# tqch/v-diffusion-torch

Hardware: AMD Instinct MI355X
Metric: train_images_per_sec (higher is better)
Workload: dtype fp32 (bf16x3 split products in the tile-engine GEMMs)

## Files before the change

v-diffusion-torch_amd/csrc/common.h:

```cpp
#pragma once
#include <hip/hip_runtime.h>
#include <stdint.h>
#include <stdio.h>
#include "../../include/vdiff_hip.h"

typedef float f32x4 __attribute__((ext_vector_type(4)));
typedef float f32x16 __attribute__((ext_vector_type(16)));

typedef float f32x2 __attribute__((ext_vector_type(2)));

#ifdef VD_PROBES
constexpr bool VD_PROBE_BUILD = true;
#else
constexpr bool VD_PROBE_BUILD = false;
#endif

void vd_set_error(const char* fmt, ...);
int vd_cu_count(void);
int vd_persistent_cus(void);
int vd_gemm_grouped_wgrad_kblk(const float* const* A, const float* const* B, float* const* C, float* const* colsum, int32_t count, int32_t M,
                               int32_t N, int32_t K, int64_t lda, int64_t ldb, int64_t ldc, int32_t splitk, float* ws, size_t ws_bytes,
                               void* stream, int64_t a_kblk, int64_t b_kblk, int32_t slabs_only);
int vd_gemm_grouped_wgrad_used_slabs(int32_t count, int32_t M, int32_t N, int32_t K, int32_t splitk);
int vd_gemm_rowblk(const vd_gemm_desc* d, int64_t a_rblk, void* stream);
// ... 14 lines not shown
__device__ __forceinline__ float vd_sigmoid(float x) { return __builtin_amdgcn_rcpf(1.0f + __expf(-x)); }

__device__ __forceinline__ void vd_philox4(uint64_t seed, uint64_t ctr, uint32_t out[4]) {
    uint32_t k0 = (uint32_t)seed, k1 = (uint32_t)(seed >> 32);
    uint32_t c0 = (uint32_t)ctr, c1 = (uint32_t)(ctr >> 32), c2 = 0x243F6A88u, c3 = 0x85A308D3u;
#pragma unroll
    for (int r = 0; r < 10; ++r) {
        uint64_t p0 = (uint64_t)0xD2511F53u * c0, p1 = (uint64_t)0xCD9E8D57u * c2;
        uint32_t n0 = (uint32_t)(p1 >> 32) ^ c1 ^ k0, n2 = (uint32_t)(p0 >> 32) ^ c3 ^ k1;
        c1 = (uint32_t)p1; c3 = (uint32_t)p0; c0 = n0; c2 = n2;
        k0 += 0x9E3779B9u; k1 += 0xBB67AE85u;
    }
    out[0] = c0; out[1] = c1; out[2] = c2; out[3] = c3;
}
__device__ __forceinline__ f32x4 vd_dropout_scale4(uint64_t seed, uint64_t vec_index, float p) {
    uint32_t r[4];
    vd_philox4(seed, vec_index, r);
    const float inv = 1.0f / (1.0f - p);
    f32x4 m;
#pragma unroll
    for (int j = 0; j < 4; ++j) m[j] = ((r[j] >> 8) * (1.0f / 16777216.0f) >= p) ? inv : 0.0f;
    return m;
}
```

v-diffusion-torch_amd/csrc/norm.hip:

```cpp
#include "common.h"
#include <stdlib.h>

namespace {

constexpr int PPC = 128;

template <bool NT>
__device__ __forceinline__ f32x4 ld_stream(const float* p) {
    if (NT) return __builtin_nontemporal_load(reinterpret_cast<const f32x4*>(p));
    return *reinterpret_cast<const f32x4*>(p);
}
template <bool NT>
__device__ __forceinline__ void st_stream(float* p, f32x4 v) {
    if (NT) __builtin_nontemporal_store(v, reinterpret_cast<f32x4*>(p));
    else *reinterpret_cast<f32x4*>(p) = v;
}

struct ReduceArgs {
    const float* x; long long ldx;
    const float* dy; long long lddy;
    const float* coef;
    int act; float p_drop; unsigned long long seed; int resample; int has_norm;
    int H, W;
    long long HW;
// ... 176 lines not shown
    const int b = idx / C, c = idx % C, g = c / (C / G);
    const float mean = stats[2 * (b * G + g)], rstd = stats[2 * (b * G + g) + 1];
    float sc = rstd * gamma[c];
    float of = beta[c] - mean * sc;
    if (film) {
        const float shift = film[(long long)b * 2 * C + c], scale = film[(long long)b * 2 * C + C + c];
        sc *= (1.f + scale);
        of = of * (1.f + scale) + shift;
    }
    float* o = coef + (long long)b * 4 * C + c;
    o[0] = sc; o[C] = of; o[2 * C] = rstd; o[3 * C] = -mean * rstd;
}

struct ApplyArgs {
    const float* x; long long ldx; const float* coef; int has_norm; int act; float p_drop; unsigned long long seed;
    int resample; float* y; long long ldy; int nimg, H, W, C;
};
struct PartArgs {
    const float* p1; int C1, ch1; const float* p2; int C2, ch2; int G; float eps;
    const float* gamma; const float* beta; const float* film; float* coef_out;
};

__device__ __forceinline__ f32x4 fwd_val(const ApplyArgs& p, f32x4 v, int pix, int c4, f32x4 sc, f32x4 of, int b) {
    if (p.has_norm) v = v * sc + of;
    if (p.act) {
#pragma unroll
        for (int j = 0; j < 4; ++j) v[j] = v[j] * vd_sigmoid(v[j]);
    }
    if (p.p_drop > 0.f) {
        const unsigned long long vi = ((unsigned long long)b * p.H * p.W + pix) * (p.C >> 2) + (c4 >> 2);
        v *= vd_dropout_scale4(p.seed, vi, p.p_drop);
    }
    return v;
}
__device__ __forceinline__ f32x4 fwd_one(const ApplyArgs& p, const float* ximg, int pix, int c4, f32x4 sc, f32x4 of, int b) {
    return fwd_val(p, *reinterpret_cast<const f32x4*>(ximg + (long long)pix * p.ldx + c4), pix, c4, sc, of, b);
}

constexpr int APIX = 64;

template <bool FROM_PARTS>
__global__ __launch_bounds__(256) void gn_apply_kernel(const ApplyArgs p, int Cb, const PartArgs q) {
    __shared__ double ps[FROM_PARTS ? 2 : 1][FROM_PARTS ? 1024 : 1];
    __shared__ float gst[FROM_PARTS ? 2 : 1][FROM_PARTS ? 256 : 1];
    const int b = blockIdx.y, c0 = blockIdx.z * Cb;
    const int cbw = min(Cb, p.C - c0);
    const int vecs = cbw >> 2, rows = 256 / vecs;
    const int r = threadIdx.x / vecs, c4 = c0 + 4 * (threadIdx.x % vecs);
    const int Ho = p.resample == VD_RS_DOWN ? p.H >> 1 : (p.resample == VD_RS_UP ? p.H << 1 : p.H);
    const int Wo = p.resample == VD_RS_DOWN ? p.W >> 1 : (p.resample == VD_RS_UP ? p.W << 1 : p.W);
    const int p0 = blockIdx.x * APIX, np = min(APIX, Ho * Wo - p0);
    f32x4 sc = {1.f, 1.f, 1.f, 1.f}, of = {0.f, 0.f, 0.f, 0.f};
    if (FROM_PARTS) {
        const int C = p.C, cg = C / q.G;
        for (int cl = threadIdx.x; cl < cbw; cl += 256) {
            const int c = c0 + cl;
// ... 746 lines not shown
```

v-diffusion-torch_amd/csrc/wino43.hip:

```cpp
#include "common.h"
#include "../../include/vdiff_hip_dgrad_planes.h"
#include <stdlib.h>
#include <type_traits>

namespace {

typedef __attribute__((address_space(3))) void* lds_ptr_t;
constexpr unsigned OOB = 0x80000000u;
constexpr int KT = 8;
constexpr int TN = 32;
constexpr int TILES = 64;
constexpr int U_STAGE = 36 * 4 * 16 * 2 * 2;
constexpr int THREADS = 512;

struct Args43 {
    const float* x; long long ldx;
    const float* U;
    float* y; long long ldy;
    int nimg, H, W, K, N;
    int items_per_img;
    int ngrp;
    int ncb, nitems;
    const float* bias; const float* res; long long ldr;
    float* stats;
// ... 473 lines not shown
    o[3] = e2 + f2;
    o[4] = e2 - f2;
    o[5] = 1.265625f * d[1] + (d[5] - 2.8125f * d[3]);
}
__device__ __forceinline__ void a6(const f32x4 (&y)[4], f32x4 (&o)[6]) {
    const f32x4 e1 = y[0] + 0.5625f * y[2], f1 = 0.75f * y[1] + 0.421875f * y[3];
    const f32x4 e2 = y[0] + 2.25f * y[2], f2 = 1.5f * y[1] + 3.375f * y[3];
    o[0] = y[0];
    o[1] = e1 + f1;
    o[2] = e1 - f1;
    o[3] = e2 + f2;
    o[4] = e2 - f2;
    o[5] = y[3];
}

__device__ __forceinline__ void st_once(float* p, f32x4 v) { *reinterpret_cast<f32x4*>(p) = v; }
struct WgT43 {
    const float* x; long long ldx; const float* dy; long long lddy;
    float* V; float* dM;
    int nimg, H, W, Cin, Cout, TW, TPI, T;
    int z0;
};

__global__ __launch_bounds__(256) void wino43_wgrad_transform_kernel(const WgT43 p) {
    const int quad = blockIdx.y * 64 + threadIdx.x, tile = blockIdx.x * 4 + threadIdx.y;
    if (tile >= p.T) return;
    const int img = tile / p.TPI, tin = tile - img * p.TPI;
    const int ty = tin / p.TW, tx = tin - ty * p.TW;
    const int c4 = 4 * quad;
    if ((int)blockIdx.z + p.z0 == 0) {
        if (c4 >= p.Cin) return;
        f32x4 R[6][6];
#pragma unroll
        for (int pr = 0; pr < 6; ++pr) {
            const int yy = 4 * ty - 1 + pr;
            f32x4 d[6];
#pragma unroll
            for (int q = 0; q < 6; ++q) {
                const int xx = 4 * tx - 1 + q;
                d[q] = f32x4{0.f, 0.f, 0.f, 0.f};
                if ((unsigned)yy < (unsigned)p.H && (unsigned)xx < (unsigned)p.W)
                    d[q] = *reinterpret_cast<const f32x4*>(p.x + ((long long)(img * p.H + yy) * p.W + xx) * p.ldx + c4);
            }
            bt6(d, R[pr]);
        }
#pragma unroll
        for (int b = 0; b < 6; ++b) {
            f32x4 col[6], o[6];
#pragma unroll
            for (int pr = 0; pr < 6; ++pr) col[pr] = R[pr][b];
            bt6(col, o);
#pragma unroll
            for (int a = 0; a < 6; ++a)
                st_once(p.V + ((long long)((tile >> 4) * 36 + 6 * a + b) * 16 + (tile & 15)) * p.Cin + c4, o[a]);
        }
    } else {
        if (c4 >= p.Cout) return;
        f32x4 R[4][6];
#pragma unroll
        for (int u = 0; u < 4; ++u) {
            f32x4 y[4];
#pragma unroll
            for (int v = 0; v < 4; ++v)
                y[v] = *reinterpret_cast<const f32x4*>(p.dy + ((long long)(img * p.H + 4 * ty + u) * p.W + 4 * tx + v) * p.lddy + c4);
            a6(y, R[u]);
        }
#pragma unroll
        for (int b = 0; b < 6; ++b) {
            const f32x4 col[4] = {R[0][b], R[1][b], R[2][b], R[3][b]};
            f32x4 o[6];
            a6(col, o);
#pragma unroll
            for (int a = 0; a < 6; ++a)
                st_once(p.dM + ((long long)((tile >> 4) * 36 + 6 * a + b) * 16 + (tile & 15)) * p.Cout + c4, o[a]);
        }
    }
}

__global__ __launch_bounds__(256) void wino43_wgrad_finish_kernel(const float* dU, const float* cs, int Cout, int Cin, int Cout_w, int Cin_w,
                                                                  float* dw, float* dbias, int accumulate) {
    const long long idx = (long long)blockIdx.x * blockDim.x + threadIdx.x;
    if (dbias && idx < Cout_w) {
        const double pv[6] = {-1.0 / 9, 8.0 / 9, 0.0, 2.0 / 9, 0.0, -1.0 / 8};
        double c = 0.0;
#pragma unroll
        for (int a = 0; a < 6; ++a)
#pragma unroll
            for (int b = 0; b < 6; ++b)
                if (pv[a] != 0.0 && pv[b] != 0.0) c += pv[a] * pv[b] * (double)cs[(long long)(6 * a + b) * Cout + idx];
        dbias[idx] = accumulate ? dbias[idx] + (float)c : (float)c;
    }
    if (idx >= (long long)Cout * Cin) return;
    const int co = (int)(idx / Cin), ci = (int)(idx - (long long)co * Cin);
    if (co >= Cout_w || ci >= Cin_w) return;
    float u[6][6];
#pragma unroll
    for (int a = 0; a < 6; ++a)
#pragma unroll
        for (int b = 0; b < 6; ++b) u[a][b] = dU[(long long)(6 * a + b) * Cout * Cin + idx];
// ... 504 lines not shown
    if (T >= (1LL << 22) || 36LL * 16 * Cin * 16 + 16LL * Cin + 256 >= 0x70000000LL / 4) return 0;
    if (128LL * Cin + 128 >= 0x70000000LL / 4 || 128LL * Cout + 128 >= 0x70000000LL / 4) return 0;
    return 1;
}

extern "C" size_t vd_conv3x3_wino43_v_floats(int32_t nimg, int32_t H, int32_t W, int32_t Cin) {
    return (size_t)36 * ((size_t)nimg * (H / 4) * (W / 4)) * Cin;
}

extern "C" size_t vd_conv3x3_wino43_fwd_planes_ws_bytes(int32_t nimg, int32_t H, int32_t W, int32_t Cin, int32_t Cout) {
    const size_t T = (size_t)nimg * (H / 4) * (W / 4);
    return ((size_t)36 * Cout * Cin + (size_t)36 * T * Cout) * sizeof(float);
}

extern "C" int vd_conv3x3_fwd_planes_preferred(int32_t nimg, int32_t H, int32_t W, int32_t Cin, int32_t Cout, int32_t training) {
    if (!vd_conv3x3_wino43_fwd_planes_supported(nimg, H, W, Cin, Cout, Cin, Cout, Cout)) return 0;
    const long long T = (long long)nimg * (H / 4) * (W / 4);
    static const long long floor_t = getenv("VD_PLANES_MIN_TILES") ? atoll(getenv("VD_PLANES_MIN_TILES")) : VD_PLANES_MIN_TILES;
    static const int inference = getenv("VD_PLANES_INFERENCE") ? atoi(getenv("VD_PLANES_INFERENCE")) : VD_PLANES_INFERENCE;
    if (T < floor_t || Cout % 256 || Cin % 16) return 0;
    return training ? VD_PLANES_TRAINING : (inference != 0);
}

extern "C" int vd_conv3x3_wino43_fwd_planes(const float* xin, int64_t ldx, const float* w_oihw, const float* bias, const float* res,
                                            int64_t ldres, float* y, int64_t ldy, int32_t nimg, int32_t H, int32_t W, int32_t Cin,
                                            int32_t Cout, float* stats_part, float* V, float* ws, size_t ws_bytes, int32_t phase, void* stream) {
    VD_REQUIRE(xin && w_oihw && y && V && ws, "vd_conv3x3_wino43_fwd_planes: null operand");
    VD_REQUIRE(vd_conv3x3_wino43_fwd_planes_supported(nimg, H, W, Cin, Cout, ldx, ldy, res ? ldres : 0),
               "vd_conv3x3_wino43_fwd_planes: unsupported geometry nimg=%d H=%d W=%d Cin=%d Cout=%d", nimg, H, W, Cin, Cout);
    VD_REQUIRE(vd_aligned16(xin) && vd_aligned16(y) && vd_aligned16(V) && vd_aligned16(ws) && (!res || vd_aligned16(res)) &&
               (!bias || vd_aligned16(bias)), "vd_conv3x3_wino43_fwd_planes: operands must be 16-byte aligned");
    VD_REQUIRE(ws_bytes >= vd_conv3x3_wino43_fwd_planes_ws_bytes(nimg, H, W, Cin, Cout), "vd_conv3x3_wino43_fwd_planes: workspace too small");
    VD_REQUIRE(phase == 7 || phase == 1 || phase == 2 || phase == 4, "vd_conv3x3_wino43_fwd_planes: phase must be 7, 1, 2 or 4");
    const int TPI = (H / 4) * (W / 4), T = nimg * TPI;
    float* Up = ws;
    float* Mb = ws + (size_t)36 * Cout * Cin;
    hipStream_t st = (hipStream_t)stream;
    if (phase & 1) {
        const long long plane = (long long)Cout * Cin;
        hipLaunchKernelGGL(wino43_pack_planes_kernel, dim3((unsigned)((plane + 255) / 256)), dim3(256), 0, st, w_oihw, Up, Cout, Cin);
        VD_LAUNCH_CHECK("wino43_pack_planes_kernel");
        WgT43 t = {};
        t.x = xin; t.ldx = ldx; t.V = V;
        t.nimg = nimg; t.H = H; t.W = W; t.Cin = Cin; t.Cout = Cout; t.TW = W / 4; t.TPI = TPI; t.T = T;
        t.z0 = 0;
        hipLaunchKernelGGL(wino43_wgrad_transform_kernel, dim3((unsigned)(T / 4), (unsigned)((Cin + 255) / 256), 1), dim3(64, 4), 0, st, t);
        VD_LAUNCH_CHECK("wino43_wgrad_transform_kernel(V)");
    }
    if (phase & 2) {
        vd_gemm_desc d = {};
        d.A = V; d.B = Up; d.C = Mb;
        d.M = T; d.N = Cout; d.K = Cin; d.a_kind = VD_ROW; d.b_kind = VD_ROW;
        d.lda = Cin; d.ldb = Cin; d.ldc = Cout;
        d.batch = 36; d.nh = 1; d.alpha = 1.f;
        d.sAb = 16LL * Cin; d.sBb = (long long)Cout * Cin; d.sCb = (long long)T * Cout;
        const int rc = vd_gemm_rowblk(&d, 36LL * 16 * Cin, stream);
        if (rc) return rc;
    }
    if (phase & 4) {
        Out43 o = {};
        o.M = Mb; o.plane = (long long)T * Cout; o.bias = bias; o.res = res; o.ldr = ldres; o.y = y; o.ldy = ldy; o.stats = stats_part;
        o.H = H; o.W = W; o.Cout = Cout; o.TW = W / 4; o.TPI = TPI; o.T = T;
        o.CT = vd_conv3x3_wino43_fwd_chunk_rows(H, W) / 16;
        hipLaunchKernelGGL(wino43_out_transform_kernel, dim3((unsigned)(T / o.CT), (unsigned)((Cout + 63) / 64)), dim3(16, 16), 0, st, o);
        VD_LAUNCH_CHECK("wino43_out_transform_kernel");
    }
    return 0;
}

extern "C" size_t vd_conv3x3_wino43_dm_floats(int32_t nimg, int32_t H, int32_t W, int32_t Cout) {
    const size_t T = (size_t)nimg * (H / 4) * (W / 4);
    return (size_t)36 * ((T + 15) / 16 * 16) * Cout;
}

extern "C" int vd_conv3x3_wino43_dy_image(const float* dy, int64_t lddy, int32_t nimg, int32_t H, int32_t W, int32_t Cout, float* dM,
                                          void* stream) {
    VD_REQUIRE(dy && dM, "vd_conv3x3_wino43_dy_image: null operand");
    VD_REQUIRE(nimg > 0 && H >= 4 && W >= 4 && H % 4 == 0 && W % 4 == 0 && Cout > 0 && Cout % 4 == 0 && lddy % 4 == 0 && lddy >= Cout,
               "vd_conv3x3_wino43_dy_image: unsupported geometry nimg=%d H=%d W=%d Cout=%d", nimg, H, W, Cout);
    VD_REQUIRE(vd_aligned16(dy) && vd_aligned16(dM), "vd_conv3x3_wino43_dy_image: operands must be 16-byte aligned");
    const long long TPI = (long long)(H / 4) * (W / 4), T = nimg * TPI;
    VD_REQUIRE(T % 4 == 0 && T < (1LL << 31) && (long long)nimg * H * W * lddy < 0x7FFFFFF0LL / 4 && T * Cout * 4 < (1LL << 40),
               "vd_conv3x3_wino43_dy_image: tile count or tensor size out of range");
    WgT43 t = {};
    t.dy = dy; t.lddy = lddy; t.dM = dM;
    t.nimg = nimg; t.H = H; t.W = W; t.Cin = Cout; t.Cout = Cout; t.TW = W / 4; t.TPI = (int)TPI; t.T = (int)T;
    t.z0 = 1;
    hipLaunchKernelGGL(wino43_wgrad_transform_kernel, dim3((unsigned)(T / 4), (unsigned)((Cout + 255) / 256), 1), dim3(64, 4), 0,
                       (hipStream_t)stream, t);
    VD_LAUNCH_CHECK("wino43_wgrad_transform_kernel(dM)");
// ... 72 lines not shown
```

v-diffusion-torch_amd/v_diffusion/_hip.py:

```python
import ctypes as C
import os
import re

import numpy as np
import torch

_HERE = os.path.dirname(os.path.abspath(__file__))
HEADER_PATH = os.path.join(os.path.dirname(os.path.dirname(_HERE)), "include", "vdiff_hip.h")
LIB_PATH = os.environ.get("VDIFF_HIP_LIB") or os.path.join(os.path.dirname(_HERE), "lib", "libvdiff_hip.so")

ROW, COL, IM2COL = 0, 1, 2
TILE_WIDE = 128256
RS_NONE, RS_DOWN, RS_UP = 0, 1, 2
OUT_TYPES = {"v": 0, "x0": 1, "eps": 2, "both": 3}
REWEIGHTS = {"constant": 0, "snr": 1, "snr_trunc": 2, "snr_1plus": 3}

_i32, _i64, _f32, _vp = C.c_int32, C.c_int64, C.c_float, C.c_void_p


class GemmDesc(C.Structure):
    _fields_ = [("A", _vp), ("B", _vp), ("C", _vp), ("bias", _vp), ("R", _vp),
                ("M", _i32), ("N", _i32), ("K", _i32), ("a_kind", _i32), ("b_kind", _i32),
                ("lda", _i64), ("ldb", _i64), ("ldc", _i64), ("ldr", _i64),
                ("batch", _i32), ("nh", _i32),
# ... 35 lines not shown
        return _BY_VALUE[ctype]
    if ret not in _RETURNS:
        raise RuntimeError(f"{HEADER_PATH}: {name}: no ctypes type for the return type `{ret}`")
    return _RETURNS[ret], [arg(q) for q in params]


def _header_signatures(path=None):
    path = path or HEADER_PATH
    if not os.path.exists(path):
        raise RuntimeError(f"{path} not found: the ctypes binding is read from the C headers of the source tree")
    with open(path) as f:
        tables = _parse_header(f.read())
    return [{name: _ctypes_of(name, *decl) for name, decl in t.items()} for t in tables]


_SIGNATURES, PROBE_EXPORTS = _header_signatures()
EXPORTS = tuple(_SIGNATURES)
EXT_HEADER_PATHS = (os.path.join(os.path.dirname(HEADER_PATH), "vdiff_hip_dgrad_planes.h"),)
_EXT_SIGNATURES = {name: sig for path in EXT_HEADER_PATHS for name, sig in _header_signatures(path)[0].items()}
EXT_EXPORTS = tuple(_EXT_SIGNATURES)
DPS_HEADER_PATHS = (os.path.join(os.path.dirname(HEADER_PATH), "vdiff_hip_dps.h"),)
_DPS_SIGNATURES = {name: sig for path in DPS_HEADER_PATHS for name, sig in _header_signatures(path)[0].items()}
DPS_EXPORTS = tuple(_DPS_SIGNATURES)

_lib = None


def lib():
    global _lib
    if _lib is None:
        if not os.path.exists(LIB_PATH):
            raise RuntimeError(
                f"{LIB_PATH} not found: build it with `python __graft_entry__.py` (or make -C v-diffusion-torch_amd/csrc). "
                "The v_diffusion hot path has no CPU/PyTorch fallback.")
        l = C.CDLL(LIB_PATH)
        for name, (res, args) in {**_SIGNATURES, **_EXT_SIGNATURES, **_DPS_SIGNATURES}.items():
            fn = getattr(l, name)
            fn.restype, fn.argtypes = res, args
        for name, (res, args) in PROBE_EXPORTS.items():
            if hasattr(l, name):
                fn = getattr(l, name)
                fn.restype, fn.argtypes = res, args
        _lib = l
    return _lib


class HipError(RuntimeError):
    pass


_CPU_TENSOR = "v_diffusion HIP op received a CPU tensor: the hot path runs on an MI355X only (no CPU fallback)"


def _check(rc, what):
    if rc != 0:
        raise HipError(f"{what} failed (rc={rc}): {lib().vd_last_error().decode(errors='replace')}")


def ptr(t):
# ... 257 lines not shown
    with _TimedName(name, 2.0 * nimg * H * W * Cout * 9 * Cin):
        _check(lib().vd_conv3x3_wino43_fwd(ptr(x), ldx, ptr(U43f), ptr(bias), ptr(res), ldres, ptr(y), ldy, nimg, H, W, Cin, Cout,
                                           ptr(stats_part), stream()), "vd_conv3x3_wino43_fwd")
    _note_bytes(name, 4.0 * (nimg * H * W * (Cin + Cout + (Cout if res is not None else 0)) + 36 * Cout * Cin))


CONV_PLANES = os.environ.get("VD_CONV_PLANES", "1")


def conv3x3_fwd_planes_preferred(nimg, H, W, Cin, Cout, training):
    return bool(lib().vd_conv3x3_fwd_planes_preferred(nimg, H, W, Cin, Cout, int(bool(training))))


def conv_planes_supported(nimg, H, W, Cin, Cout, ldx, ldy, ldres=0, training=False):
    if CONV_PLANES == "0" or not (WINO and WINO43_FWD):
        return False
    if not lib().vd_conv3x3_wino43_fwd_planes_supported(nimg, H, W, Cin, Cout, ldx, ldy, ldres):
        return False
    if training and not wgrad43_supported(nimg, H, W, Cin, Cout, Cin, Cout):
        return False
    return CONV_PLANES == "2" or conv3x3_fwd_planes_preferred(nimg, H, W, Cin, Cout, training)


def conv3x3_wino43_fwd_planes(x, ldx, w, bias, y, ldy, nimg, H, W, Cin, Cout, res=None, ldres=0, stats_part=None, v=None):
    nv = lib().vd_conv3x3_wino43_v_floats(nimg, H, W, Cin)
    if v is None:
        v = workspace(nv * 4, x.device, "planes_v")
    assert v.numel() >= nv and w.is_contiguous() and tuple(w.shape) == (Cout, Cin, 3, 3)
    ws = workspace(lib().vd_conv3x3_wino43_fwd_planes_ws_bytes(nimg, H, W, Cin, Cout), x.device, "planes")
    args = (ptr(x), ldx, ptr(w), ptr(bias), ptr(res), ldres, ptr(y), ldy, nimg, H, W, Cin, Cout, ptr(stats_part), ptr(v), ws.data_ptr(),
            ws.numel() * 4)
    phase = lambda ph: _check(lib().vd_conv3x3_wino43_fwd_planes(*args, ph, stream()), "vd_conv3x3_wino43_fwd_planes")
    if PROFILE is None:
        phase(7)
        return
    T = nimg * (H // 4) * (W // 4)
    with _TimedBytes("wino43_wgrad_transform_kernel", 4.0 * nimg * H * W * Cin * (1 + 2.25)):
        phase(1)
    with _TimedTile("gemm_dma_kernel<{tile}, 0, 0, false, {kt}>", 2.0 * 36 * T * Cout * Cin):
        phase(2)
    _note_bytes(PROFILE[-1][0], 4.0 * 36.0 * (T * (Cin + Cout) + Cout * Cin))
    with _TimedBytes("wino43_out_transform_kernel", 4.0 * (36.0 * T * Cout + nimg * H * W * Cout * (2 if res is not None else 1))):
        phase(4)


DGRAD_PLANES = os.environ.get("VD_DGRAD_PLANES", "1")


def dgrad_planes_supported(nimg, H, W, Cin, Cout, lddy, lddx):
    if DGRAD_PLANES == "0" or not (WINO and WINO43):
        return False
    if lddy % 4 or not lib().vd_conv3x3_wino43_dgrad_planes_supported(nimg, H, W, Cin, Cout, lddx):
        return False
    if not wgrad43_supported(nimg, H, W, Cin, Cout, Cin, lddy):
        return False
# ... 633 lines not shown
```

v-diffusion-torch_amd/v_diffusion/engine.py:

```python
import collections
import contextlib
import math

import torch

from . import _hip as H

GROUPS = 32
EPS = 1e-6
THIN = 8


def _ld(t):
    return t.stride(2)


def _chk(t):
    B, Hh, Ww, C = t.shape
    ld = t.stride(2)
    assert t.stride(3) == 1 and t.stride(1) == Ww * ld and t.stride(0) == Hh * Ww * ld, "not an NHWC view"
    return B, Hh, Ww, C, ld


def _splitk(M, N, K, n=1):
# ... 203 lines not shown
        return torch.empty(H.stats_part_numel(nimg, HW, C), dtype=torch.float32, device=ref.device)

    @staticmethod
    def _parts(part, C, HW, rows=None):
        if part is None:
            return None
        return [(part, C, HW // (rows or (H.last_row_tile() // 2)))]

    def _norm(self, x, x_parts, gn, film, act, p_drop, seed, rs, y, B, Hh, Ww, C):
        coef = self._new(x, B, 4, C)
        stats = None
        if x_parts is not None and H.GN_FOLD and max(k for _, _, k in x_parts) <= H.GN_FOLD_MAX_CHUNKS:
            H.gn_apply_from_partials(x, _ld(x), x_parts, gn.weight, gn.bias, film, act, p_drop, seed, rs, y, _ld(y), B, Hh, Ww, C, coef,
                                     GROUPS, EPS)
            return coef
        if x_parts is not None:
            H.gn_coef_from_partials(x_parts, B, Hh * Ww, gn.weight, gn.bias, film, coef, GROUPS, EPS)
        else:
            stats = self._new(x, B, GROUPS, 2)
            H.gn_stats(x, _ld(x), B, Hh * Ww, C, stats, GROUPS, EPS)
        H.gn_apply(x, _ld(x), stats, gn.weight, gn.bias, film, act, p_drop, seed, rs, y, _ld(y), B, Hh, Ww, C, coef, GROUPS)
        return coef

    def _wgrad(self, dy, x, dw, db, M, N, K, lda, ldb, ldc):
        if self._wq is None or not H.GROUPED_WGRAD:
            H.gemm(dy, x, dw, M, N, K, a_kind=H.COL, b_kind=H.COL, lda=lda, ldb=ldb, ldc=ldc, splitk=_splitk(M, N, K), colsum=db)
            return
        key = (M, N, K, lda, ldb, ldc, db is not None)
        q = self._wq.setdefault(key, [])
        q.append((dy, x, dw, db))
        if len(q) == H.GROUP_MAX:
            self._wgrad_flush_key(key)

    def _cwgrad(self, x, ldx, dy, lddy, *args, v=None, **kw):
        if v is not None:
            kw["v"] = v
        side = self._side
        if side is None:
            return H.conv3x3_wgrad(x, ldx, dy, lddy, *args, **kw)
        side.wait_stream(torch.cuda.current_stream())
        (x if v is None else v).record_stream(side)
        dy.record_stream(side)
        with torch.cuda.stream(side):
            H.conv3x3_wgrad(x, ldx, dy, lddy, *args, **kw)

    def _conv_bwd_planes(self, w, v, dy, lddy, dx, lddx, B, Hh, Ww, Cin, Cout, gw, gb):
# ... 90 lines not shown
        if pk is None:
            pk = ConvPacks(ws, need_d, self._conv_geoms(*geom) if geom is not None else [])
            while len(self._pack_lru) >= self.PACK_STATES_MAX:
                self._pack_lru.pop(next(iter(self._pack_lru)))
        self._pack_lru[key] = self._packs = pk
        pk.repack()
        return pk

    @property
    def packs(self):
        return self._packs

    @contextlib.contextmanager
    def fixed_weights(self):
        self._fixed = {}
        try:
            yield
        finally:
            self._fixed = None

    def _layer(self, w):
        return self._packs.layers.get(id(w), _NO_PACK) if self._packs is not None else _NO_PACK

    def _conv(self, x, ldx, w, bias, y, ldy, B, Hh, Ww, Cin, Cout, dgrad=False, res=None, ldres=0, stats_part=None, keep_v=None):
        pk, p = self._packs, self._layer(w)
        if not dgrad and p is not _NO_PACK and pk.wino and H.conv_planes_supported(B, Hh, Ww, Cin, Cout, ldx, ldy, ldres if res is not None else 0,
                                                                                 training=keep_v is not None):
            v = None
            if keep_v is not None:
                v = torch.empty(36 * B * (Hh // 4) * (Ww // 4) * Cin, dtype=torch.float32, device=x.device)
                keep_v.append(v)
            H.conv3x3_wino43_fwd_planes(x, ldx, w, bias, y, ldy, B, Hh, Ww, Cin, Cout, res=res, ldres=ldres, stats_part=stats_part, v=v)
            return H.wino43_fwd_chunk_rows(Hh, Ww)
        if not dgrad and p.u43f is not None and H.wino43_fwd_supported(B, Hh, Ww, Cin, Cout, ldx, ldy, ldres if res is not None else 0):
            H.conv3x3_wino43_fwd(x, ldx, p.u43f, bias, y, ldy, B, Hh, Ww, Cin, Cout, res=res, ldres=ldres, stats_part=stats_part)
            return H.wino43_fwd_chunk_rows(Hh, Ww)
        if dgrad and p.u43 is not None and H.wino43_supported(B, Hh, Ww, Cout, Cin, ldx, ldy):
            assert res is None and bias is None and stats_part is None
            H.conv3x3_dgrad_wino43(x, ldx, p.u43, y, ldy, B, Hh, Ww, Cout, Cin)
            return None
        if p is not _NO_PACK and pk.wino and H.wino_supported(B, Hh, Ww, Cin, Cout, ldx, ldy, ldres if res is not None else 0):
            U = p.ud if dgrad else p.uf
            if U is None:
                U = pk.image(w, dgrad)
            H.conv3x3_wino(x, ldx, U, bias, y, ldy, B, Hh, Ww, Cin, Cout, res=res, ldres=ldres, stats_part=stats_part)
            return H.last_row_tile() // 2
        H.conv3x3(x, ldx, self._pack_d(w) if dgrad else self._pack_f(w), bias, y, ldy, B, Hh, Ww, Cin, Cout, res=res, ldres=ldres,
                  stats_part=stats_part)
        return H.last_row_tile() // 2

    def _pack_f(self, w, cin_p=None):
        p = self._layer(w)
        if p.wf is not None:
            return p.wf
        cache = self._fixed
# ... 120 lines not shown
            nb = len(mods)
            out = self._new(ta, nb, B, c2)
            H.gemm(ta, W, out, B, c2, E, a_kind=H.ROW, b_kind=H.ROW, lda=E, ldb=E, ldc=c2, bias=bv, sBias=c2, batch=nb,
                   sA=(0, 0), sB=(c2 * E, 0), sC=(B * c2, 0))
            films[c2], stacks[c2] = out, W
        if tape is not None:
            tape["film_w"] = stacks
        return films

    def _film_bwd(self, dfilms, stacks, dta):
        B, E = dta.shape
        for c2, df in dfilms.items():
            nb, W = df.shape[0], stacks[c2]
            P = self._new(dta, nb, B * E)
            H.gemm(df, W, P, B, E, c2, a_kind=H.ROW, b_kind=H.COL, lda=c2, ldb=E, ldc=E, batch=nb, sA=(B * c2, 0), sB=(c2 * E, 0),
                   sC=(B * E, 0))
            H.colsum(P, B * E, nb, B * E, dta.view(-1), accumulate=True)

    def _res_fwd(self, blk, x, films, dest, p_drop, seed, tape, x_parts=None):
        mod, prefix = blk.res, blk.res_prefix
        B, Hh, Ww, Cin, ldx = _chk(x)
        Cout, rs = blk.cout, blk.rs
        Ho, Wo = H._resampled(Hh, Ww, rs)
        a1 = self._new(x, B, Ho, Wo, Cin)
        coef1 = self._norm(x, x_parts, mod.norm1, None, 1, 0.0, 0, rs, a1, B, Hh, Ww, Cin)
        h1 = self._new(x, B, Ho, Wo, Cout)
        ph = self._part(x, B, Ho * Wo, Cout)
        v1, v2 = ([], []) if tape is not None else (None, None)
        rows = self._conv(a1, Cin, mod.conv1.weight, mod.conv1.bias, h1, Cout, B, Ho, Wo, Cin, Cout, stats_part=ph, keep_v=v1)
        h1_parts = self._parts(ph, Cout, Ho * Wo, rows)
        c2, fi = blk.film
        film = films[c2][fi]
        a2 = self._new(x, B, Ho, Wo, Cout)
        coef2 = self._norm(h1, h1_parts, mod.norm2, film, 1, p_drop, seed, H.RS_NONE, a2, B, Ho, Wo, Cout)
        if rs != H.RS_NONE:
            xs = self._new(x, B, Ho, Wo, Cin)
            H.gn_apply(x, ldx, None, None, None, None, 0, 0.0, 0, rs, xs, Cin, B, Hh, Ww, Cin, None, GROUPS)
        else:
            xs = x
        has_skip = Cin != Cout
        if has_skip:
            sk = self._new(x, B, Ho, Wo, Cout)
            w = mod.skip.weight
            H.gemm(xs, w, sk, B * Ho * Wo, Cout, Cin, a_kind=H.ROW, b_kind=H.ROW, lda=_ld(xs), ldb=Cin, ldc=Cout, bias=mod.skip.bias)
        else:
            sk = xs
        pd = self._part(x, B, Ho * Wo, Cout)
        rows = self._conv(a2, Cout, mod.conv2.weight, mod.conv2.bias, dest, _ld(dest), B, Ho, Wo, Cout, Cout, res=sk,
                          ldres=_ld(sk), stats_part=pd, keep_v=v2)
        out_parts = self._parts(pd, Cout, Ho * Wo, rows)
        if tape is not None:
            tape[prefix] = dict(x=x, coef1=coef1, a1=None if v1 else a1, h1=h1, coef2=coef2, a2=None if v2 else a2, film=film,
                                xs=xs if has_skip else None, seed=seed, p=p_drop, v1=v1[0] if v1 else None, v2=v2[0] if v2 else None)
        return out_parts

    def _res_bwd(self, blk, ctx, dy, dx, dx_accumulate, ta, dfilms, G):
        mod = blk.res
        only_dx = G is None
        g = _NO_GRADS if only_dx else {s: G[name] for s, name in blk.res_names.items()}
        x, a1, h1, a2, film = ctx["x"], ctx["a1"], ctx["h1"], ctx["a2"], ctx["film"]
        B, Hh, Ww, Cin, ldx = _chk(x)
        _, Ho, Wo, Cout, lddy = _chk(dy)
        rs = blk.rs
        da2 = self._new(x, B, Ho, Wo, Cout)
        if not self._conv_bwd_planes(mod.conv2.weight, ctx["v2"], dy, lddy, da2, Cout, B, Ho, Wo, Cout, Cout, g["conv2.weight"], g["conv2.bias"]):
            if not only_dx:
                self._cwgrad(a2, Cout, dy, lddy, B, Ho, Wo, Cout, Cout, g["conv2.weight"], Cout, Cout, dbias=g["conv2.bias"], v=ctx["v2"])
            self._conv(dy, lddy, mod.conv2.weight, None, da2, Cout, B, Ho, Wo, Cout, Cout, dgrad=True)
        dh1 = self._new(x, B, Ho, Wo, Cout)
        c2, fi = blk.film
        dfilm = dfilms[c2][0 if only_dx else fi]
        H.gn_apply_bwd(da2, Cout, h1, Cout, ctx["coef2"], mod.norm2.weight, mod.norm2.bias, film, 1, ctx["p"], ctx["seed"],
# ... 386 lines not shown
```

Before: 2358.

## Fuse GroupNorm/SiLU/dropout apply into Winograd input transform for residual convs

Adds a planes-path Winograd forward variant that applies the group-norm affine, SiLU and dropout inside the V (input) transform kernel, reading the raw pre-norm activation directly. The residual block computes only the norm coefficients from partials and skips materialising the normalized activation tensors a1/a2, which removes one full read-and-write pass per conv. In exchange the transform kernel does more ALU work per loaded element, including Philox dropout, and is specialised via templated mode variants. It is enabled by default through an environment flag.

New measurement: 2374, median of 2. About the same (+0.7%).

```diff
diff --git a/include/vdiff_hip_conv_norm.h b/include/vdiff_hip_conv_norm.h
--- /dev/null
+++ b/include/vdiff_hip_conv_norm.h
@@ -0,0 +1,18 @@
+#ifndef VDIFF_HIP_CONV_NORM_H
+#define VDIFF_HIP_CONV_NORM_H
+#include <stddef.h>
+#include <stdint.h>
+
+#ifdef __cplusplus
+extern "C" {
+#endif
+
+int vd_conv3x3_wino43_fwd_planes_norm(const float* xin, int64_t ldx, const float* w_oihw, const float* bias, const float* res, int64_t ldres,
+                                      float* y, int64_t ldy, int32_t nimg, int32_t H, int32_t W, int32_t Cin, int32_t Cout, float* stats_part,
+                                      float* V, float* ws, size_t ws_bytes, const float* coef, int32_t act, float p_drop, uint64_t seed,
+                                      int32_t phase, void* stream);
+
+#ifdef __cplusplus
+}
+#endif
+#endif
diff --git a/v-diffusion-torch_amd/csrc/common.h b/v-diffusion-torch_amd/csrc/common.h
--- a/v-diffusion-torch_amd/csrc/common.h
+++ b/v-diffusion-torch_amd/csrc/common.h
@@ -60,3 +60,17 @@
     for (int j = 0; j < 4; ++j) m[j] = ((r[j] >> 8) * (1.0f / 16777216.0f) >= p) ? inv : 0.0f;
     return m;
 }
+
+__device__ __forceinline__ f32x4 vd_gn_fwd_val(f32x4 v, f32x4 sc, f32x4 of, int has_norm, int act, float p_drop, uint64_t seed, int b, int H,
+                                               int W, int C, int pix, int c4) {
+    if (has_norm) v = v * sc + of;
+    if (act) {
+#pragma unroll
+        for (int j = 0; j < 4; ++j) v[j] = v[j] * vd_sigmoid(v[j]);
+    }
+    if (p_drop > 0.f) {
+        const unsigned long long vi = ((unsigned long long)b * H * W + pix) * (C >> 2) + (c4 >> 2);
+        v *= vd_dropout_scale4(seed, vi, p_drop);
+    }
+    return v;
+}
diff --git a/v-diffusion-torch_amd/csrc/norm.hip b/v-diffusion-torch_amd/csrc/norm.hip
--- a/v-diffusion-torch_amd/csrc/norm.hip
+++ b/v-diffusion-torch_amd/csrc/norm.hip
@@ -222,16 +222,7 @@
 };
 
 __device__ __forceinline__ f32x4 fwd_val(const ApplyArgs& p, f32x4 v, int pix, int c4, f32x4 sc, f32x4 of, int b) {
-    if (p.has_norm) v = v * sc + of;
-    if (p.act) {
-#pragma unroll
-        for (int j = 0; j < 4; ++j) v[j] = v[j] * vd_sigmoid(v[j]);
-    }
-    if (p.p_drop > 0.f) {
-        const unsigned long long vi = ((unsigned long long)b * p.H * p.W + pix) * (p.C >> 2) + (c4 >> 2);
-        v *= vd_dropout_scale4(p.seed, vi, p.p_drop);
-    }
-    return v;
+    return vd_gn_fwd_val(v, sc, of, p.has_norm, p.act, p.p_drop, p.seed, b, p.H, p.W, p.C, pix, c4);
 }
 __device__ __forceinline__ f32x4 fwd_one(const ApplyArgs& p, const float* ximg, int pix, int c4, f32x4 sc, f32x4 of, int b) {
     return fwd_val(p, *reinterpret_cast<const f32x4*>(ximg + (long long)pix * p.ldx + c4), pix, c4, sc, of, b);
diff --git a/v-diffusion-torch_amd/csrc/wino43.hip b/v-diffusion-torch_amd/csrc/wino43.hip
--- a/v-diffusion-torch_amd/csrc/wino43.hip
+++ b/v-diffusion-torch_amd/csrc/wino43.hip
@@ -1,5 +1,6 @@
 #include "common.h"
 #include "../../include/vdiff_hip_dgrad_planes.h"
+#include "../../include/vdiff_hip_conv_norm.h"
 #include <stdlib.h>
 #include <type_traits>
 
@@ -519,6 +520,60 @@
     int z0;
 };
 
+struct VNorm43 { const float* coef; int act; float p_drop; unsigned long long seed; };
+
+template <int MODE>
+__device__ __forceinline__ void wino43_v_tile(const WgT43& p, const VNorm43& n, int tile, int img, int ty, int tx, int c4) {
+    f32x4 sc = {1.f, 1.f, 1.f, 1.f}, of = {0.f, 0.f, 0.f, 0.f};
+    if (MODE >= 0 && (MODE & 1)) {
+        const float* cf = n.coef + (long long)img * 4 * p.Cin;
+        sc = *reinterpret_cast<const f32x4*>(cf + c4);
+        of = *reinterpret_cast<const f32x4*>(cf + p.Cin + c4);
+    }
+    if (MODE >= 0 && (MODE & 4)) __builtin_assume(n.p_drop > 0.f);
+    f32x4 R[6][6];
+#pragma unroll
+    for (int pr = 0; pr < 6; ++pr) {
+        const int yy = 4 * ty - 1 + pr;
+        f32x4 d[6];
+        if (MODE < 0) {
+#pragma unroll
+            for (int q = 0; q < 6; ++q) {
+                const int xx = 4 * tx - 1 + q;
+                d[q] = f32x4{0.f, 0.f, 0.f, 0.f};
+                if ((unsigned)yy < (unsigned)p.H && (unsigned)xx < (unsigned)p.W)
+                    d[q] = *reinterpret_cast<const f32x4*>(p.x + ((long long)(img * p.H + yy) * p.W + xx) * p.ldx + c4);
+            }
+        } else {
+            const int yc = min(max(yy, 0), p.H - 1);
+#pragma unroll
+            for (int q = 0; q < 6; ++q) {
+                const int xc = min(max(4 * tx - 1 + q, 0), p.W - 1);
+                d[q] = *reinterpret_cast<const f32x4*>(p.x + ((long long)(img * p.H + yc) * p.W + xc) * p.ldx + c4);
+            }
+#pragma unroll
+            for (int q = 0; q < 6; ++q) {
+                const int xx = 4 * tx - 1 + q, xc = min(max(xx, 0), p.W - 1);
+                const f32x4 a = vd_gn_fwd_val(d[q], sc, of, MODE & 1, MODE & 2, (MODE & 4) ? n.p_drop : 0.f, n.seed, img, p.H, p.W, p.Cin,
+                                              yc * p.W + xc, c4);
+                d[q] = (yy == yc && xx == xc) ? a : f32x4{0.f, 0.f, 0.f, 0.f};
+                asm("" : "+v"(d[q]));
+            }
+        }
+        bt6(d, R[pr]);
+    }
+#pragma unroll
+    for (int b = 0; b < 6; ++b) {
+        f32x4 col[6], o[6];
+#pragma unroll
+        for (int pr = 0; pr < 6; ++pr) col[pr] = R[pr][b];
+        bt6(col, o);
+#pragma unroll
+        for (int a = 0; a < 6; ++a)
+            st_once(p.V + ((long long)((tile >> 4) * 36 + 6 * a + b) * 16 + (tile & 15)) * p.Cin + c4, o[a]);
+    }
+}
+
 __global__ __launch_bounds__(256) void wino43_wgrad_transform_kernel(const WgT43 p) {
     const int quad = blockIdx.y * 64 + threadIdx.x, tile = blockIdx.x * 4 + threadIdx.y;
     if (tile >= p.T) return;
@@ -527,30 +582,7 @@
     const int c4 = 4 * quad;
     if ((int)blockIdx.z + p.z0 == 0) {
         if (c4 >= p.Cin) return;
-        f32x4 R[6][6];
-#pragma unroll
-        for (int pr = 0; pr < 6; ++pr) {
-            const int yy = 4 * ty - 1 + pr;
-            f32x4 d[6];
-#pragma unroll
-            for (int q = 0; q < 6; ++q) {
-                const int xx = 4 * tx - 1 + q;
-                d[q] = f32x4{0.f, 0.f, 0.f, 0.f};
-                if ((unsigned)yy < (unsigned)p.H && (unsigned)xx < (unsigned)p.W)
-                    d[q] = *reinterpret_cast<const f32x4*>(p.x + ((long long)(img * p.H + yy) * p.W + xx) * p.ldx + c4);
-            }
-            bt6(d, R[pr]);
-        }
-#pragma unroll
-        for (int b = 0; b < 6; ++b) {
-            f32x4 col[6], o[6];
-#pragma unroll
-            for (int pr = 0; pr < 6; ++pr) col[pr] = R[pr][b];
-            bt6(col, o);
-#pragma unroll
-            for (int a = 0; a < 6; ++a)
-                st_once(p.V + ((long long)((tile >> 4) * 36 + 6 * a + b) * 16 + (tile & 15)) * p.Cin + c4, o[a]);
-        }
+        wino43_v_tile<-1>(p, VNorm43{}, tile, img, ty, tx, c4);
     } else {
         if (c4 >= p.Cout) return;
         f32x4 R[4][6];
@@ -572,6 +604,20 @@
                 st_once(p.dM + ((long long)((tile >> 4) * 36 + 6 * a + b) * 16 + (tile & 15)) * p.Cout + c4, o[a]);
         }
     }
+}
+
+template <int MODE>
+__global__ __launch_bounds__(256) void wino43_wgrad_transform_norm_kernel(const WgT43 p, const VNorm43 n) {
+    const int c4 = 4 * (blockIdx.y * 64 + threadIdx.x), tile = blockIdx.x * 4 + threadIdx.y;
+    if (tile >= p.T || c4 >= p.Cin) return;
+    const int img = tile / p.TPI, tin = tile - img * p.TPI;
+    const int ty = tin / p.TW;
+    wino43_v_tile<MODE>(p, n, tile, img, ty, tin - ty * p.TW, c4);
+}
+
+template <int MODE>
+static void launch_v_norm(dim3 grid, hipStream_t st, const WgT43& t, const VNorm43& n) {
+    hipLaunchKernelGGL(wino43_wgrad_transform_norm_kernel<MODE>, grid, dim3(64, 4), 0, st, t, n);
 }
 
 __global__ __launch_bounds__(256) void wino43_wgrad_finish_kernel(const float* dU, const float* cs, int Cout, int Cin, int Cout_w, int Cin_w,
@@ -1122,16 +1168,17 @@
     return training ? VD_PLANES_TRAINING : (inference != 0);
 }
 
-extern "C" int vd_conv3x3_wino43_fwd_planes(const float* xin, int64_t ldx, const float* w_oihw, const float* bias, const float* res,
-                                            int64_t ldres, float* y, int64_t ldy, int32_t nimg, int32_t H, int32_t W, int32_t Cin,
-                                            int32_t Cout, float* stats_part, float* V, float* ws, size_t ws_bytes, int32_t phase, void* stream) {
-    VD_REQUIRE(xin && w_oihw && y && V && ws, "vd_conv3x3_wino43_fwd_planes: null operand");
+static int fwd_planes_impl(const char* who, const float* xin, int64_t ldx, const float* w_oihw, const float* bias, const float* res,
+                           int64_t ldres, float* y, int64_t ldy, int32_t nimg, int32_t H, int32_t W, int32_t Cin, int32_t Cout,
+                           float* stats_part, float* V, float* ws, size_t ws_bytes, int32_t phase, void* stream, const VNorm43* n) {
+    VD_REQUIRE(xin && w_oihw && y && V && ws, "%s: null operand", who);
     VD_REQUIRE(vd_conv3x3_wino43_fwd_planes_supported(nimg, H, W, Cin, Cout, ldx, ldy, res ? ldres : 0),
-               "vd_conv3x3_wino43_fwd_planes: unsupported geometry nimg=%d H=%d W=%d Cin=%d Cout=%d", nimg, H, W, Cin, Cout);
+               "%s: unsupported geometry nimg=%d H=%d W=%d Cin=%d Cout=%d", who, nimg, H, W, Cin, Cout);
     VD_REQUIRE(vd_aligned16(xin) && vd_aligned16(y) && vd_aligned16(V) && vd_aligned16(ws) && (!res || vd_aligned16(res)) &&
-               (!bias || vd_aligned16(bias)), "vd_conv3x3_wino43_fwd_planes: operands must be 16-byte aligned");
-    VD_REQUIRE(ws_bytes >= vd_conv3x3_wino43_fwd_planes_ws_bytes(nimg, H, W, Cin, Cout), "vd_conv3x3_wino43_fwd_planes: workspace too small");
-    VD_REQUIRE(phase == 7 || phase == 1 || phase == 2 || phase == 4, "vd_conv3x3_wino43_fwd_planes: phase must be 7, 1, 2 or 4");
+               (!bias || vd_aligned16(bias)) && (!n || vd_aligned16(n->coef)), "%s: operands must be 16-byte aligned", who);
+    VD_REQUIRE(ws_bytes >= vd_conv3x3_wino43_fwd_planes_ws_bytes(nimg, H, W, Cin, Cout), "%s: workspace too small", who);
+    VD_REQUIRE(phase == 7 || phase == 1 || phase == 2 || phase == 4, "%s: phase must be 7, 1, 2 or 4", who);
+    VD_REQUIRE(!n || (n->p_drop >= 0.f && n->p_drop < 1.f), "%s: p_drop must be in [0, 1)", who);
     const int TPI = (H / 4) * (W / 4), T = nimg * TPI;
     float* Up = ws;
     float* Mb = ws + (size_t)36 * Cout * Cin;
@@ -1144,8 +1191,23 @@
         t.x = xin; t.ldx = ldx; t.V = V;
         t.nimg = nimg; t.H = H; t.W = W; t.Cin = Cin; t.Cout = Cout; t.TW = W / 4; t.TPI = TPI; t.T = T;
         t.z0 = 0;
-        hipLaunchKernelGGL(wino43_wgrad_transform_kernel, dim3((unsigned)(T / 4), (unsigned)((Cin + 255) / 256), 1), dim3(64, 4), 0, st, t);
-        VD_LAUNCH_CHECK("wino43_wgrad_transform_kernel(V)");
+        if (n) {
+            const dim3 grid((unsigned)(T / 4), (unsigned)((Cin + 255) / 256));
+            switch ((n->coef ? 1 : 0) | (n->act ? 2 : 0) | (n->p_drop > 0.f ? 4 : 0)) {
+                case 0: launch_v_norm<0>(grid, st, t, *n); break;
+                case 1: launch_v_norm<1>(grid, st, t, *n); break;
+                case 2: launch_v_norm<2>(grid, st, t, *n); break;
+                case 3: launch_v_norm<3>(grid, st, t, *n); break;
+                case 4: launch_v_norm<4>(grid, st, t, *n); break;
+                case 5: launch_v_norm<5>(grid, st, t, *n); break;
+                case 6: launch_v_norm<6>(grid, st, t, *n); break;
+                default: launch_v_norm<7>(grid, st, t, *n); break;
+            }
+            VD_LAUNCH_CHECK("wino43_wgrad_transform_norm_kernel");
+        } else {
+            hipLaunchKernelGGL(wino43_wgrad_transform_kernel, dim3((unsigned)(T / 4), (unsigned)((Cin + 255) / 256), 1), dim3(64, 4), 0, st, t);
+            VD_LAUNCH_CHECK("wino43_wgrad_transform_kernel(V)");
+        }
     }
     if (phase & 2) {
         vd_gemm_desc d = {};
@@ -1166,6 +1228,22 @@
         VD_LAUNCH_CHECK("wino43_out_transform_kernel");
     }
     return 0;
+}
+
+extern "C" int vd_conv3x3_wino43_fwd_planes(const float* xin, int64_t ldx, const float* w_oihw, const float* bias, const float* res,
+                                            int64_t ldres, float* y, int64_t ldy, int32_t nimg, int32_t H, int32_t W, int32_t Cin,
+                                            int32_t Cout, float* stats_part, float* V, float* ws, size_t ws_bytes, int32_t phase, void* stream) {
+    return fwd_planes_impl("vd_conv3x3_wino43_fwd_planes", xin, ldx, w_oihw, bias, res, ldres, y, ldy, nimg, H, W, Cin, Cout, stats_part, V, ws,
+                           ws_bytes, phase, stream, nullptr);
+}
+
+extern "C" int vd_conv3x3_wino43_fwd_planes_norm(const float* xin, int64_t ldx, const float* w_oihw, const float* bias, const float* res,
+                                                 int64_t ldres, float* y, int64_t ldy, int32_t nimg, int32_t H, int32_t W, int32_t Cin,
+                                                 int32_t Cout, float* stats_part, float* V, float* ws, size_t ws_bytes, const float* coef,
+                                                 int32_t act, float p_drop, uint64_t seed, int32_t phase, void* stream) {
+    const VNorm43 n = {coef, act, p_drop, seed};
+    return fwd_planes_impl("vd_conv3x3_wino43_fwd_planes_norm", xin, ldx, w_oihw, bias, res, ldres, y, ldy, nimg, H, W, Cin, Cout, stats_part, V,
+                           ws, ws_bytes, phase, stream, &n);
 }
 
 extern "C" size_t vd_conv3x3_wino43_dm_floats(int32_t nimg, int32_t H, int32_t W, int32_t Cout) {
diff --git a/v-diffusion-torch_amd/v_diffusion/_hip.py b/v-diffusion-torch_amd/v_diffusion/_hip.py
--- a/v-diffusion-torch_amd/v_diffusion/_hip.py
+++ b/v-diffusion-torch_amd/v_diffusion/_hip.py
@@ -81,6 +81,9 @@
 DPS_HEADER_PATHS = (os.path.join(os.path.dirname(HEADER_PATH), "vdiff_hip_dps.h"),)
 _DPS_SIGNATURES = {name: sig for path in DPS_HEADER_PATHS for name, sig in _header_signatures(path)[0].items()}
 DPS_EXPORTS = tuple(_DPS_SIGNATURES)
+CONV_NORM_HEADER_PATHS = (os.path.join(os.path.dirname(HEADER_PATH), "vdiff_hip_conv_norm.h"),)
+_CONV_NORM_SIGNATURES = {name: sig for path in CONV_NORM_HEADER_PATHS for name, sig in _header_signatures(path)[0].items()}
+CONV_NORM_EXPORTS = tuple(_CONV_NORM_SIGNATURES)
 
 _lib = None
 
@@ -93,7 +96,7 @@
                 f"{LIB_PATH} not found: build it with `python __graft_entry__.py` (or make -C v-diffusion-torch_amd/csrc). "
                 "The v_diffusion hot path has no CPU/PyTorch fallback.")
         l = C.CDLL(LIB_PATH)
-        for name, (res, args) in {**_SIGNATURES, **_EXT_SIGNATURES, **_DPS_SIGNATURES}.items():
+        for name, (res, args) in {**_SIGNATURES, **_EXT_SIGNATURES, **_DPS_SIGNATURES, **_CONV_NORM_SIGNATURES}.items():
             fn = getattr(l, name)
             fn.restype, fn.argtypes = res, args
         for name, (res, args) in PROBE_EXPORTS.items():
@@ -397,7 +400,10 @@
     return CONV_PLANES == "2" or conv3x3_fwd_planes_preferred(nimg, H, W, Cin, Cout, training)
 
 
-def conv3x3_wino43_fwd_planes(x, ldx, w, bias, y, ldy, nimg, H, W, Cin, Cout, res=None, ldres=0, stats_part=None, v=None):
+CONV_NORM = os.environ.get("VD_CONV_NORM", "1") != "0"
+
+
+def conv3x3_wino43_fwd_planes(x, ldx, w, bias, y, ldy, nimg, H, W, Cin, Cout, res=None, ldres=0, stats_part=None, v=None, norm=None):
     nv = lib().vd_conv3x3_wino43_v_floats(nimg, H, W, Cin)
     if v is None:
         v = workspace(nv * 4, x.device, "planes_v")
@@ -405,7 +411,13 @@
     ws = workspace(lib().vd_conv3x3_wino43_fwd_planes_ws_bytes(nimg, H, W, Cin, Cout), x.device, "planes")
     args = (ptr(x), ldx, ptr(w), ptr(bias), ptr(res), ldres, ptr(y), ldy, nimg, H, W, Cin, Cout, ptr(stats_part), ptr(v), ws.data_ptr(),
             ws.numel() * 4)
-    phase = lambda ph: _check(lib().vd_conv3x3_wino43_fwd_planes(*args, ph, stream()), "vd_conv3x3_wino43_fwd_planes")
+    if norm is None:
+        phase = lambda ph: _check(lib().vd_conv3x3_wino43_fwd_planes(*args, ph, stream()), "vd_conv3x3_wino43_fwd_planes")
+    else:
+        coef, act, p_drop, seed = norm
+        assert coef is None or coef.numel() >= nimg * 4 * Cin
+        nargs = args + (ptr(coef), int(act), float(p_drop), int(seed))
+        phase = lambda ph: _check(lib().vd_conv3x3_wino43_fwd_planes_norm(*nargs, ph, stream()), "vd_conv3x3_wino43_fwd_planes_norm")
     if PROFILE is None:
         phase(7)
         return
diff --git a/v-diffusion-torch_amd/v_diffusion/engine.py b/v-diffusion-torch_amd/v_diffusion/engine.py
--- a/v-diffusion-torch_amd/v_diffusion/engine.py
+++ b/v-diffusion-torch_amd/v_diffusion/engine.py
@@ -249,6 +249,11 @@
         H.gn_apply(x, _ld(x), stats, gn.weight, gn.bias, film, act, p_drop, seed, rs, y, _ld(y), B, Hh, Ww, C, coef, GROUPS)
         return coef
 
+    def _norm_coef(self, x, x_parts, gn, film, B, Hh, Ww, C):
+        coef = self._new(x, B, 4, C)
+        H.gn_coef_from_partials(x_parts, B, Hh * Ww, gn.weight, gn.bias, film, coef, GROUPS, EPS)
+        return coef
+
     def _wgrad(self, dy, x, dw, db, M, N, K, lda, ldb, ldc):
         if self._wq is None or not H.GROUPED_WGRAD:
             H.gemm(dy, x, dw, M, N, K, a_kind=H.COL, b_kind=H.COL, lda=lda, ldb=ldb, ldc=ldc, splitk=_splitk(M, N, K), colsum=db)
@@ -385,15 +390,41 @@
     def _layer(self, w):
         return self._packs.layers.get(id(w), _NO_PACK) if self._packs is not None else _NO_PACK
 
-    def _conv(self, x, ldx, w, bias, y, ldy, B, Hh, Ww, Cin, Cout, dgrad=False, res=None, ldres=0, stats_part=None, keep_v=None):
+    def _fwd_planes(self, w, B, Hh, Ww, Cin, Cout, ldx, ldy, ldres, training):
+        return self._layer(w) is not _NO_PACK and self._packs.wino and H.conv_planes_supported(B, Hh, Ww, Cin, Cout, ldx, ldy, ldres,
+                                                                                               training=training)
+
+    def _norm_in_conv(self, x, x_parts, rs, w, B, Hh, Ww, Cin, Cout, ldy, ldres, training):
+        return (x_parts is not None and x.data_ptr() % 16 == 0 and self._layer(w) is not _NO_PACK and self._packs.wino
+                and self._norm_in_conv_rule(rs, B, Hh, Ww, Cin, Cout, _ld(x), ldy, ldres, training))
+
+    @staticmethod
+    def _norm_in_conv_rule(rs, B, Hh, Ww, Cin, Cout, ldx, ldy, ldres, training):
+        return (H.CONV_NORM and rs == H.RS_NONE and H.conv_planes_supported(B, Hh, Ww, Cin, Cout, Cin, ldy, ldres, training=training)
+                and H.conv_planes_supported(B, Hh, Ww, Cin, Cout, ldx, ldy, ldres, training=training))
+
+    def norm_in_conv_plan(self, B, H0, W0, training=True):
+        out = []
+        for b in self.plan:
+            if b.res is None:
+                continue
+            lh, lw = H._resampled(*self._res_of(b.level, H0, W0), b.rs)
+            if self._norm_in_conv_rule(b.rs, B, lh, lw, b.cin, b.cout, b.cin, b.cout, 0, training):
+                out.append((b.res_prefix, "conv1"))
+            if self._norm_in_conv_rule(H.RS_NONE, B, lh, lw, b.cout, b.cout, b.cout, b.cout, b.cout, training):
+                out.append((b.res_prefix, "conv2"))
+        return out
+
+    def _conv(self, x, ldx, w, bias, y, ldy, B, Hh, Ww, Cin, Cout, dgrad=False, res=None, ldres=0, stats_part=None, keep_v=None, norm=None):
         pk, p = self._packs, self._layer(w)
-        if not dgrad and p is not _NO_PACK and pk.wino and H.conv_planes_supported(B, Hh, Ww, Cin, Cout, ldx, ldy, ldres if res is not None else 0,
-                                                                                 training=keep_v is not None):
+        planes = not dgrad and self._fwd_planes(w, B, Hh, Ww, Cin, Cout, ldx, ldy, ldres if res is not None else 0, keep_v is not None)
+        assert norm is None or planes, "a norm was left to a convolution that does not go through planes"
+        if planes:
             v = None
             if keep_v is not None:
                 v = torch.empty(36 * B * (Hh // 4) * (Ww // 4) * Cin, dtype=torch.float32, device=x.device)
                 keep_v.append(v)
-            H.conv3x3_wino43_fwd_planes(x, ldx, w, bias, y, ldy, B, Hh, Ww, Cin, Cout, res=res, ldres=ldres, stats_part=stats_part, v=v)
+            H.conv3x3_wino43_fwd_planes(x, ldx, w, bias, y, ldy, B, Hh, Ww, Cin, Cout, res=res, ldres=ldres, stats_part=stats_part, v=v, norm=norm)
             return H.wino43_fwd_chunk_rows(Hh, Ww)
         if not dgrad and p.u43f is not None and H.wino43_fwd_supported(B, Hh, Ww, Cin, Cout, ldx, ldy, ldres if res is not None else 0):
             H.conv3x3_wino43_fwd(x, ldx, p.u43f, bias, y, ldy, B, Hh, Ww, Cin, Cout, res=res, ldres=ldres, stats_part=stats_part)
@@ -560,23 +591,36 @@
         B, Hh, Ww, Cin, ldx = _chk(x)
         Cout, rs = blk.cout, blk.rs
         Ho, Wo = H._resampled(Hh, Ww, rs)
-        a1 = self._new(x, B, Ho, Wo, Cin)
-        coef1 = self._norm(x, x_parts, mod.norm1, None, 1, 0.0, 0, rs, a1, B, Hh, Ww, Cin)
+        training = tape is not None
+        has_skip = Cin != Cout
+        a1 = a2 = None
+        if self._norm_in_conv(x, x_parts, rs, mod.conv1.weight, B, Ho, Wo, Cin, Cout, Cout, 0, training):
+            coef1 = self._norm_coef(x, x_parts, mod.norm1, None, B, Hh, Ww, Cin)
+            cin1, ld1, norm1 = x, ldx, (coef1, 1, 0.0, 0)
+        else:
+            a1 = self._new(x, B, Ho, Wo, Cin)
+            coef1 = self._norm(x, x_parts, mod.norm1, None, 1, 0.0, 0, rs, a1, B, Hh, Ww, Cin)
+            cin1, ld1, norm1 = a1, Cin, None
         h1 = self._new(x, B, Ho, Wo, Cout)
         ph = self._part(x, B, Ho * Wo, Cout)
-        v1, v2 = ([], []) if tape is not None else (None, None)
-        rows = self._conv(a1, Cin, mod.conv1.weight, mod.conv1.bias, h1, Cout, B, Ho, Wo, Cin, Cout, stats_part=ph, keep_v=v1)
+        v1, v2 = ([], []) if training else (None, None)
+        rows = self._conv(cin1, ld1, mod.conv1.weight, mod.conv1.bias, h1, Cout, B, Ho, Wo, Cin, Cout, stats_part=ph, keep_v=v1, norm=norm1)
         h1_parts = self._parts(ph, Cout, Ho * Wo, rows)
         c2, fi = blk.film
         film = films[c2][fi]
-        a2 = self._new(x, B, Ho, Wo, Cout)
-        coef2 = self._norm(h1, h1_parts, mod.norm2, film, 1, p_drop, seed, H.RS_NONE, a2, B, Ho, Wo, Cout)
+        ldsk = Cout if has_skip else (ldx if rs == H.RS_NONE else Cin)
+        if self._norm_in_conv(h1, h1_parts, H.RS_NONE, mod.conv2.weight, B, Ho, Wo, Cout, Cout, _ld(dest), ldsk, training):
+            coef2 = self._norm_coef(h1, h1_parts, mod.norm2, film, B, Ho, Wo, Cout)
+            cin2, norm2 = h1, (coef2, 1, p_drop, seed)
+        else:
+            a2 = self._new(x, B, Ho, Wo, Cout)
+            coef2 = self._norm(h1, h1_parts, mod.norm2, film, 1, p_drop, seed, H.RS_NONE, a2, B, Ho, Wo, Cout)
+            cin2, norm2 = a2, None
         if rs != H.RS_NONE:
             xs = self._new(x, B, Ho, Wo, Cin)
             H.gn_apply(x, ldx, None, None, None, None, 0, 0.0, 0, rs, xs, Cin, B, Hh, Ww, Cin, None, GROUPS)
         else:
             xs = x
-        has_skip = Cin != Cout
         if has_skip:
             sk = self._new(x, B, Ho, Wo, Cout)
             w = mod.skip.weight
@@ -584,8 +628,9 @@
         else:
             sk = xs
         pd = self._part(x, B, Ho * Wo, Cout)
-        rows = self._conv(a2, Cout, mod.conv2.weight, mod.conv2.bias, dest, _ld(dest), B, Ho, Wo, Cout, Cout, res=sk,
-                          ldres=_ld(sk), stats_part=pd, keep_v=v2)
+        assert _ld(sk) == ldsk
+        rows = self._conv(cin2, Cout, mod.conv2.weight, mod.conv2.bias, dest, _ld(dest), B, Ho, Wo, Cout, Cout, res=sk,
+                          ldres=ldsk, stats_part=pd, keep_v=v2, norm=norm2)
         out_parts = self._parts(pd, Cout, Ho * Wo, rows)
         if tape is not None:
             tape[prefix] = dict(x=x, coef1=coef1, a1=None if v1 else a1, h1=h1, coef2=coef2, a2=None if v2 else a2, film=film,
```
